# acrlabs/kube-scheduler-rs-reference

Measured on AMD Instinct MI355X. Metric: pod x node predicate evals/s, higher is better.
Workload: dtype int64

## Files before the change

kube_scheduler_rs_reference_amd/csrc/kernels_fused.hpp:

```cpp
#pragma once
#include <hip/hip_ext.h>
#include <hip/hip_runtime.h>
#include <stdint.h>

#include <type_traits>

#include "eval_request.hpp"
#include "kernarg.hpp"
#include "kernels_direct.hpp"
#include "tile_index.hpp"
#include "tile_launch.hpp"

#ifndef KSCHED_STORE_POLICY
#define KSCHED_STORE_POLICY 6
#endif
#ifndef KSCHED_STORE_ALT
#define KSCHED_STORE_ALT(it) ((it) == 7u)
#endif
#ifndef KSCHED_PROFILE
#define KSCHED_PROFILE 0
#endif
#if defined(KSCHED_FUSED_NUM_VGPR)
#define KSCHED_FUSED_WPE_ATTR __attribute__((amdgpu_num_vgpr(KSCHED_FUSED_NUM_VGPR)))
#elif defined(KSCHED_FUSED_WPE)
// ... 76 lines not shown
                if (eager == 1u) bnd = select_one_pod<5, 3>(sa, pod);
                else if (eager == 2u) bnd = select_one_pod<5, 5>(sa, pod);
                else if (eager == 3u) bnd = select_one_pod<5, 2>(sa, pod);
                else bnd = select_one_pod<5, 1>(sa, pod);
                sa.binding[pod] = bnd;
            }
            if (a.trace && threadIdx.x == 0u)
                atomicOr((unsigned long long *)&a.trace[(size_t)b * 8u + 7u], (unsigned long long)((wall_clock64() - t_in) << 8));
        }
        asm volatile("" : "+v"(tid) : : "memory");
    }
    const uint32_t lane = tid & 63u;
    const uint32_t wave = __builtin_amdgcn_readfirstlane(tid >> 6);
    const uint32_t stage_rank = (PICK == 1 && !(a.debug & 0x10000u)) ? wave - pick_waves : wave;
    const uint32_t stage_waves = kFusedWaves - pick_waves;
    const bool tracer = a.trace && tid == (PICK == 1 ? (kFusedWaves - 1u) * 64u : 0u);
    auto stamp = [&](uint32_t i) {
        if (tracer) a.trace[(size_t)b * 8u + i] = wall_clock64();
    };
    stamp(0);
    const uint32_t c_lo = chunk * a.unit_q + min(chunk, a.unit_rem);
    const uint32_t c_n = a.unit_q + (chunk < a.unit_rem ? 1u : 0u);
    uint32_t u = c_lo + (wave * c_n) / kFusedWaves;
    uint32_t u_hi = c_lo + ((wave + 1u) * c_n) / kFusedWaves;
    const uint32_t u_stride = a.u_stride;
    if (u_stride != 8u) {
        u = (a.wave_major ? wave * a.chunks + chunk : chunk * kFusedWaves + wave) * 8u;
        u_hi = a.units;
    }

    int64_t rc = 0, rm = 0;
    uint32_t s0 = 0, s1 = 0, s2 = 0, s3 = 0, s4 = 0, s5 = 0, s6 = 0, s7 = 0;
    uint64_t tol = 0;
    uint32_t d0 = 0, d1 = 0, d2 = 0, d3 = 0, d4 = 0;
    uint64_t ar = 0;
    auto issue_ops = [&](uint32_t pod) {
        const uint32_t pc = min(pod, a.p - 1u);
        if constexpr (PICK == 2) {
            static_assert(kPickAttempts == 5, "five draw registers");
            const size_t last = (size_t)a.p * kPickAttempts - 1u;
            const size_t f0 = (size_t)(pod - lane) * kPickAttempts + lane;
            asm volatile("global_load_dword %0, %1, off" : "=v"(d0) : "v"(sa.samples + min(f0, last)) : "memory");
            asm volatile("global_load_dword %0, %1, off" : "=v"(d1) : "v"(sa.samples + min(f0 + 64u, last)) : "memory");
            asm volatile("global_load_dword %0, %1, off" : "=v"(d2) : "v"(sa.samples + min(f0 + 128u, last)) : "memory");
            asm volatile("global_load_dword %0, %1, off" : "=v"(d3) : "v"(sa.samples + min(f0 + 192u, last)) : "memory");
            asm volatile("global_load_dword %0, %1, off" : "=v"(d4) : "v"(sa.samples + min(f0 + 256u, last)) : "memory");
        }
        if (FIT) {
            asm volatile("global_load_dwordx2 %0, %1, off" : "=v"(rc) : "v"(g_pcpu + pc) : "memory");
            asm volatile("global_load_dwordx2 %0, %1, off" : "=v"(rm) : "v"(g_pmem + pc) : "memory");
        }
        if (SEL) {
#define KSCHED_LOAD_SEL(K, DST)                                                                                                   \
    asm volatile("global_load_dword %0, %1, off"                                                                                  \
                 : "=v"(DST)                                                                                                      \
                 : "v"((uint32_t)K < a.nkeys ? g_psel + (size_t)K * a.p + pc : reinterpret_cast<const uint32_t *>(a.zero64)) \
                 : "memory")
            KSCHED_LOAD_SEL(0, s0);
            KSCHED_LOAD_SEL(1, s1);
            KSCHED_LOAD_SEL(2, s2);
            KSCHED_LOAD_SEL(3, s3);
            KSCHED_LOAD_SEL(4, s4);
            KSCHED_LOAD_SEL(5, s5);
            KSCHED_LOAD_SEL(6, s6);
            KSCHED_LOAD_SEL(7, s7);
#undef KSCHED_LOAD_SEL
        }
        if (TAINT) {
            const uint64_t *tp = a.has_tol ? g_ptol + pc : a.zero64;
            asm volatile("global_load_dwordx2 %0, %1, off" : "=v"(tol) : "v"(tp) : "memory");
        }
    };
#define KSCHED_WAIT_OPS(N)                                                                                                            \
    asm volatile("s_waitcnt vmcnt(%c11)"                                                                                              \
                 : "+v"(rc), "+v"(rm), "+v"(s0), "+v"(s1), "+v"(s2), "+v"(s3), "+v"(s4), "+v"(s5), "+v"(s6), "+v"(s7), "+v"(tol)  \
                 : "n"(N)                                                                                                             \
                 : "memory")
#define KSCHED_WAIT_OPS_PICK(N)                                                                                                       \
    asm volatile("s_waitcnt vmcnt(%c17)"                                                                                              \
                 : "+v"(rc), "+v"(rm), "+v"(s0), "+v"(s1), "+v"(s2), "+v"(s3), "+v"(s4), "+v"(s5), "+v"(s6), "+v"(s7), "+v"(tol), \
                   "+v"(d0), "+v"(d1), "+v"(d2), "+v"(d3), "+v"(d4), "+v"(ar)                                                     \
                 : "n"(N)                                                                                                             \
                 : "memory")
    const int64_t *s_cpu = reinterpret_cast<const int64_t *>(smem + a.off_aux);
    const int64_t *s_mem = s_cpu + kAuxTreeWords;
    const uint2 *s_cnt_cpu = reinterpret_cast<const uint2 *>(s_cpu + 2u * kAuxTreeWords);
    const uint2 *s_cnt_mem = s_cnt_cpu + kCntEntries;
    uint4 *s_fit = reinterpret_cast<uint4 *>(smem + a.off_fit) + wave * 64u;
    uint4 *s_lab = reinterpret_cast<uint4 *>(smem + a.off_lab) + wave * 64u;
    uint2 *s_trow = reinterpret_cast<uint2 *>(smem + a.off_trow) + wave * 64u;
    typedef __attribute__((address_space(3))) uint8_t lds_u8;
    lds_u8 *const lds = (lds_u8 *)smem;
    uint2 *s_lrec = reinterpret_cast<uint2 *>(smem + a.off_lrec) + wave * 64u;
    constexpr uint32_t kListCap = 8u;

    const uint32_t quad = (lane & 31u) >> 2;
    const uint32_t wp = ((0xCCu >> quad) & 1u) * 4u + (lane & 3u);
    const uint32_t sub = (lane >> 5) * 4u + ((0x31130220u >> (4u * quad)) & 15u);
    const uint32_t w0 = tile * kTileWords + 2u * wp;
    const bool has0 = w0 < a.pitch, has1 = w0 + 1u < a.pitch;
    const bool tile_full = (tile + 1u) * kTileWords <= a.pitch;
    const bool taint_inline = a.ngroups <= 4u;
    const uint8_t *Tb = smem + wp * 16u;
    const uint8_t *Tb_cpu = Tb + a.row_cpu * 128u;
    auto ldoff = [&](uint32_t off) -> u32x4 { return *reinterpret_cast<const u32x4 *>(Tb + off); };
    auto ldrow = [&](uint32_t row) -> u32x4 { return ldoff(row * 128u); };
    auto lo16 = [](uint32_t x) { return x & 0xFFFFu; };
    auto hi16 = [](uint32_t x) { return x >> 16; };
    const uint8_t *fit_lane = reinterpret_cast<const uint8_t *>(s_fit + sub) + wp;
    const uint2 *lab_lane = reinterpret_cast<const uint2 *>(s_lab + sub);
    const uint2 *trow_lane = s_trow + sub;
    auto opaque = [](uint32_t x) -> uint32_t {
        asm volatile("" : "+v"(x));
        return x;
    };
    auto lrec_of = [&](uint32_t it) -> uint2 { return (s_lrec + opaque(sub) + it * 8u)[0]; };
    auto list_mask = [&](uint32_t j, uint32_t rec, uint32_t bound, uint32_t wp) -> u32x4 {
        const uint32_t noff = a.off_list + j * kListBytes + kTileNodes * 4u;
        const uint32_t first = rec & 0xFFFFu, count = rec >> 16;
        u32x4 m = {0u, 0u, 0u, 0u};
        const uint32_t n_e = (bound != 0xFFFFFFFFu) ? bound : ((count == 0xFFFFu) ? 0u : count);
        for (uint32_t e = 0; e < n_e; ++e) {
            const uint32_t node = *(const __attribute__((address_space(3))) uint16_t *)(lds + noff + min(first + e, (uint32_t)kTileNodes - 1u) * 2u);
            const bool hit = e < count && (node >> 7) == wp;
            const uint32_t bit = hit ? (1u << (node & 31u)) : 0u, w = (node >> 5) & 3u;
            m.x |= (w == 0u) ? bit : 0u;
            m.y |= (w == 1u) ? bit : 0u;
            m.z |= (w == 2u) ? bit : 0u;
            m.w |= (w == 3u) ? bit : 0u;
        }
        const uint32_t all = (count == 0xFFFFu) ? 0xFFFFFFFFu : 0u;
        m.x |= all, m.y |= all, m.z |= all, m.w |= all;
        return m;
    };
    auto apply_lists = [&](u32x4 f, const uint2 lr, uint32_t bound) -> u32x4 {
        static_assert(kMaxListKeys == 2 && kListRecBytes == 8, "one 32-bit record slot per list key");
        const uint32_t r[2] = {lr.x, lr.y};
        const uint32_t wp_o = opaque(wp);
#pragma unroll
        for (uint32_t j = 0; j < 4; ++j)
            if (j < a.nlist) f &= list_mask(j, r[j], bound, wp_o);
        return f;
    };

    struct Rows {
        u32x4 c0, m0, l0, l1, l2, l3, t0, t1, t2, t3, x0, x1, x2, x3;
    };
    auto load_extra = [&](const uint2 r2, Rows &R) {
        R.x0 = ldoff(lo16(r2.x));
        R.x1 = ldoff(hi16(r2.x));
        R.x2 = ldoff(lo16(r2.y));
        R.x3 = ldoff(hi16(r2.y));
    };
    auto load_rows = [&](const uint32_t cc, const uint32_t cm, const uint2 lb, const uint2 tr, Rows &R) {
        if (FIT) {
            R.c0 = *reinterpret_cast<const u32x4 *>(Tb_cpu + cc * 128u);
            R.m0 = *reinterpret_cast<const u32x4 *>(Tb_cpu + cm * 128u + (uint32_t)kFitRows * 128u);
        } else {
            R.c0 = ldrow(a.row_valid);
        }
        if (SEL) {
            R.l0 = ldoff(lo16(lb.x));
            R.l1 = ldoff(hi16(lb.x));
            R.l2 = ldoff(lo16(lb.y));
            R.l3 = ldoff(hi16(lb.y));
        }
// ... 37 lines not shown
#elif KSCHED_STORE_POLICY == 2
        asm volatile("global_store_dwordx4 %0, %1, %2 sc1\n\ts_nop 1" ::"v"(voff), "v"(f), "s"(base) : "memory");
#elif KSCHED_STORE_POLICY == 3
        asm volatile("global_store_dwordx4 %0, %1, %2 sc0 sc1\n\ts_nop 1" ::"v"(voff), "v"(f), "s"(base) : "memory");
#elif KSCHED_STORE_POLICY == 4
        asm volatile("global_store_dwordx4 %0, %1, %2 sc1 nt\n\ts_nop 1" ::"v"(voff), "v"(f), "s"(base) : "memory");
#elif KSCHED_STORE_POLICY == 5
        asm volatile("global_store_dwordx4 %0, %1, %2 sc0 sc1 nt\n\ts_nop 1" ::"v"(voff), "v"(f), "s"(base) : "memory");
#elif KSCHED_STORE_POLICY == 1
        __builtin_nontemporal_store(f, reinterpret_cast<u32x4_a8 *>(reinterpret_cast<uint8_t *>(base) + voff));
#else
        *reinterpret_cast<u32x4_a8 *>(reinterpret_cast<uint8_t *>(base) + voff) = f;
#endif
    };
    auto uniform64 = [](uint64_t x) -> uint64_t {
        const uint32_t hi = (uint32_t)__builtin_amdgcn_readfirstlane((int)(uint32_t)(x >> 32)), lo = (uint32_t)__builtin_amdgcn_readfirstlane((int)(uint32_t)x);
        return ((uint64_t)hi << 32) | (uint64_t)lo;
    };
    uint64_t rb_feas = 0, rb_fit = 0;
    auto combine_store = [&](uint32_t it, const Rows &R, bool extra) {
        const uint64_t step = (uint64_t)it * step_bytes;
        u32x4 f = fit_of(R);
        if (WANT_FIT) store_rel(rb_fit + step, lane_off, f);
        if (SEL) f = ((f & R.l0) & R.l1) & (R.l2 & R.l3);
        if (SEL && extra) f = ((f & R.x0) & R.x1) & (R.x2 & R.x3);
        if (TAINT) f = ((f & R.t0) & R.t1) & (R.t2 & R.t3);
        store_rel(rb_feas + step, lane_off, f, KSCHED_STORE_ALT(it));
    };

    auto emit_checked = [&](uint32_t pod, uint32_t it, bool over) {
        const bool live = pod < a.p && has0;
        Rows R;
        if (LIST) {
            uint32_t sub_o = sub, wp_o = wp;
            asm volatile("" : "+v"(sub_o), "+v"(wp_o));
            const uint8_t *fit_o = reinterpret_cast<const uint8_t *>(s_fit + sub_o) + wp_o;
            const uint2 *lab_o = reinterpret_cast<const uint2 *>(s_lab + sub_o);
            load_rows(FIT ? (uint32_t)(fit_o + it * 128u)[0] : 0u, FIT ? (uint32_t)(fit_o + it * 128u)[8] : 0u, (lab_o + it * 16u)[0],
                      TAINT ? (s_trow + sub_o + it * 8u)[0] : make_uint2(0u, 0u), R);
            load_extra((lab_o + it * 16u)[1], R);
        } else {
            load_rows(rec_cc(it), rec_cm(it), rec_lb(it), rec_tr(it), R);
            if (SEL) load_extra(rec_lx(it), R);
        }
        u32x4 f = fit_of(R);
        const size_t o = (size_t)pod * a.pitch + w0;
        auto store = [&](uint64_t *dst) {
            if (has1) store16(dst, o, f);
            else dst[o] = ((uint64_t)f.y << 32) | f.x;
        };
        if (WANT_FIT && live) store(out_fit);
        if (SEL) {
            if (!over) {
                f = ((f & R.l0) & R.l1) & (R.l2 & R.l3);
                f = ((f & R.x0) & R.x1) & (R.x2 & R.x3);
            } else if (live) {
                for (uint32_t k = 0; k < a.nkeys; ++k) {
                    if (LIST && a.lab_meta[k] == kLabList) continue;
                    const uint32_t s = g_psel[(size_t)k * a.p + pod];
                    if (s != 0u) f &= ldrow((s <= a.lab_meta[32u + k]) ? (a.lab_meta[k] + s - 1u) : a.row_zero);
                }
            }
        }
        if (TAINT) {
            if (taint_inline) {
                f = ((f & R.t0) & R.t1) & (R.t2 & R.t3);
            } else if (live) {
                const uint64_t t = a.has_tol ? g_ptol[pod] : 0ull;
                for (uint32_t g = 0; g < a.ngroups; ++g) f &= ldrow(a.row_taint + 16u * g + (uint32_t)((t >> (4u * g)) & 15ull));
            }
        }
        if (LIST) {
            __builtin_amdgcn_sched_barrier(0);
            f = apply_lists(f, lrec_of(it), 0xFFFFFFFFu);
        }
        if (live && out_feas && !(a.debug & 1u)) store(out_feas);
    };

    bool extra_any = false, list_any = false;
    uint32_t list_bound = 0;
    uint32_t pick_bits = 0;
    typedef __attribute__((address_space(3))) uint32_t lds_u32;
    lds_u32 *const s_park = (lds_u32 *)(lds + a.off_park) + wave * (kPickAttempts * 64u);
    auto phase1 = [&](uint32_t pod0) -> uint64_t {
        uint2 cnt_c = make_uint2(0u, 0u), cnt_m = make_uint2(0u, 0u);
        if (FIT) {
            uint32_t lc = 0, lm = 0;
            if (!(a.debug & 2u)) {
                uint32_t kc = 1, km = 1;
#pragma unroll
                for (uint32_t level = 0; level < 10; ++level) {
                    const int64_t vc = s_cpu[kc], vm = s_mem[km];
                    kc = 2u * kc + ((vc < rc) ? 1u : 0u);
                    km = 2u * km + ((vm < rm) ? 1u : 0u);
                }
                lc = kc - (uint32_t)kTileNodes;
                lm = km - (uint32_t)kTileNodes;
                lc += (lc == (uint32_t)kTileNodes - 1u && s_cpu[0] < rc) ? 1u : 0u;
                lm += (lm == (uint32_t)kTileNodes - 1u && s_mem[0] < rm) ? 1u : 0u;
            }
            const uint2 cc = s_cnt_cpu[lc], cm = s_cnt_mem[lm];
            s_fit[lane] = make_uint4(cc.x, cc.y, cm.x, cm.y);
            cnt_c = cc;
            cnt_m = cm;
        }
        const uint32_t rv = a.row_valid * 128u;
        uint32_t cnt = 0;
        if (SEL) {
            const uint32_t rv2 = rv | (rv << 16);
            s_lab[lane] = make_uint4(rv2, rv2, rv2, rv2);
            uint16_t *const slots = reinterpret_cast<uint16_t *>(s_lab + lane);
            uint16_t *slot = slots;
            const uint32_t sv[8] = {s0, s1, s2, s3, s4, s5, s6, s7};
#pragma unroll
            for (uint32_t k = 0; k < 8; ++k) {
                const uint32_t s = sv[k];
                if (s != 0u && !(LIST && ((a.list_mask8 >> k) & 1u))) {
                    *slot++ = (uint16_t)(min(s, a.lab_mx1[k]) * 128u + a.lab_off[k]);
                }
            }
            cnt = (uint32_t)(slot - slots);
            if (a.nkeys > 8u) {
                const uint32_t pc = min(pod0 + lane, a.p - 1u);
                for (uint32_t k = 8; k < a.nkeys; ++k) {
                    if (LIST && a.lab_meta[k] == kLabList) continue;
                    cnt += (g_psel[(size_t)k * a.p + pc] != 0u) ? 9u : 0u;
                }
            }
        }
        uint32_t lmax = 0;
        if (LIST) {
            uint32_t lv[kMaxListKeys] = {0u, 0u};
#pragma unroll
            for (uint32_t j = 0; j < kMaxListKeys; ++j) {
                if (j >= a.nlist) continue;
                const uint32_t col = a.list_col[j];
                if (col < 8u) {
                    uint32_t v = s0;
                    v = (col == 1u) ? s1 : v;
                    v = (col == 2u) ? s2 : v;
                    v = (col == 3u) ? s3 : v;
                    v = (col == 4u) ? s4 : v;
                    v = (col == 5u) ? s5 : v;
                    v = (col == 6u) ? s6 : v;
                    v = (col == 7u) ? s7 : v;
                    lv[j] = v;
                } else {
                    lv[j] = g_psel[(size_t)col * a.p + min(pod0 + lane, a.p - 1u)];
                }
            }
            uint32_t rec[kMaxListKeys] = {0xFFFF0000u, 0xFFFF0000u};
            bool any = false;
#pragma unroll
            for (uint32_t j = 0; j < kMaxListKeys; ++j) {
                rec[j] = 0xFFFF0000u;
                const uint32_t s = lv[j];
                if (j < a.nlist && s != 0u) {
                    const uint32_t voff = a.off_list + j * kListBytes;
                    auto val_at = [&](uint32_t e) -> uint32_t { return *(const __attribute__((address_space(3))) uint32_t *)(lds + voff + e * 4u); };
                    auto lower = [&](uint32_t key) -> uint32_t {
                        uint32_t base = 0;
#pragma unroll
                        for (uint32_t half = (uint32_t)kTileNodes / 2u; half >= 1u; half >>= 1) base += (val_at(base + half - 1u) < key) ? half : 0u;
                        return base + ((val_at(base) < key) ? 1u : 0u);
                    };
                    const uint32_t lo = lower(s);
                    uint32_t cnt = 0;
                    bool run = true;
#pragma unroll
                    for (uint32_t e = 0; e <= kListCap; ++e) {
                        run = run && lo + e < (uint32_t)kTileNodes && val_at(min(lo + e, (uint32_t)kTileNodes - 1u)) == s;
                        cnt += run ? 1u : 0u;
                    }
                    if (cnt > kListCap) cnt = lower(s + 1u) - lo;
                    rec[j] = lo | (cnt << 16);
                    lmax = max(lmax, cnt);
                    any = true;
                }
            }
            s_lrec[lane] = make_uint2(rec[0], rec[1]);
            list_any = __ballot(any) != 0ull;
#pragma unroll
            for (uint32_t d = 32; d >= 1; d >>= 1) lmax = max(lmax, (uint32_t)__shfl_xor((int)lmax, d, 64));
            list_bound = (uint32_t)__builtin_amdgcn_readfirstlane((int)lmax);
        }
        if (TAINT) {
            uint32_t t[4];
#pragma unroll
            for (uint32_t g = 0; g < 4; ++g)
                t[g] = (g < a.ngroups) ? (a.row_taint + 16u * g + (uint32_t)((tol >> (4u * g)) & 15ull)) * 128u : rv;
            s_trow[lane] = make_uint2(t[0] | (t[1] << 16), t[2] | (t[3] << 16));
        }
        if constexpr (PICK == 2) {
            const uint4 slots = SEL ? s_lab[lane] : make_uint4(0u, 0u, 0u, 0u);
            s_park[lane] = d0;
            s_park[64u + lane] = d1;
            s_park[128u + lane] = d2;
            s_park[192u + lane] = d3;
            s_park[256u + lane] = d4;
            uint32_t dv[kPickAttempts];
#pragma unroll
            for (uint32_t i = 0; i < kPickAttempts; ++i) dv[i] = s_park[lane * kPickAttempts + i];
            uint32_t bits = 0;
#pragma unroll
            for (uint32_t i = 0; i < kPickAttempts; ++i) {
                const uint32_t l = dv[i] - tile * (uint32_t)kTileNodes;
                if (l < (uint32_t)kTileNodes && !(a.debug & 0x8000000u)) {
                    const uint32_t wofs = (l >> 5) << 2, sub = l >> 7;
                    auto word = [&](uint32_t off) -> uint32_t { return *(lds_u32 *)(lds + off + wofs); };
                    uint32_t v;
                    if (FIT) {
                        const uint32_t sh = (sub & 3u) * 8u;
                        const uint32_t bc = ((sub < 4u ? cnt_c.x : cnt_c.y) >> sh) & 0xFFu, bm = ((sub < 4u ? cnt_m.x : cnt_m.y) >> sh) & 0xFFu;
                        v = word((a.row_cpu + bc) * 128u) & word((a.row_cpu + (uint32_t)kFitRows + bm) * 128u);
                    } else {
                        v = word(rv);
                    }
                    if (SEL)
                        v &= word(slots.x & 0xFFFFu) & word(slots.x >> 16) & word(slots.y & 0xFFFFu) & word(slots.y >> 16) & word(slots.z & 0xFFFFu) &
                             word(slots.z >> 16) & word(slots.w & 0xFFFFu) & word(slots.w >> 16);
                    bits |= ((v >> (l & 31u)) & 1u) << i;
                }
            }
            pick_bits = bits;
        }
        extra_any = __ballot(cnt > 4u) != 0ull;
        const uint64_t over = __ballot(cnt > 8u || (LIST && lmax > kListCap));
        __builtin_amdgcn_fence(__ATOMIC_RELEASE, "wavefront");
        __builtin_amdgcn_wave_barrier();
        return over;
    };

    constexpr int kFastStores = 8 * (WANT_FIT ? 2 : 1);

    constexpr uint32_t kPrefetchRounds = 6;
    auto prefetch_rounds = [&]() {
        if (!(FIT || SEL || TAINT) || a.off_pf == 0xFFFFFFFFu || u + u_stride * (kPrefetchRounds + 2u) < u_hi || (a.debug & 0x20000000u)) return;
        const uint32_t dump = (uint32_t)__builtin_amdgcn_readfirstlane((int)a.off_pf);
        const uint32_t li = opaque(lane);
#pragma unroll 1
        for (uint32_t r = 1; r <= kPrefetchRounds; ++r) {
            const uint32_t pu = u + u_stride * r;
            if (pu >= u_hi) break;
            const uint32_t pod0 = pu * 8u;
            const uint32_t pe = a.p - 1u;
            const uint32_t e8 = min(pod0 + (li & 3u) * 16u, pe);
            uint64_t a64 = reinterpret_cast<uint64_t>(a.zero64);
            if (FIT && li < 4u) a64 = reinterpret_cast<uint64_t>(g_pcpu + e8);
            if (FIT && li >= 4u && li < 8u) a64 = reinterpret_cast<uint64_t>(g_pmem + e8);
            if (SEL && a.nkeys && li >= 8u && li < 24u) {
                const uint32_t k = min((li - 8u) >> 1, min(a.nkeys, 8u) - 1u);
                a64 = reinterpret_cast<uint64_t>(g_psel + (size_t)k * a.p + min(pod0 + (li & 1u) * 32u, pe));
            }
            if (PICK == 2 && li >= 24u && li < 34u) {
                a64 = reinterpret_cast<uint64_t>(sa.samples + min((size_t)pod0 * kPickAttempts + (li - 24u) * 32u, (size_t)a.p * kPickAttempts - 1u));
            }
            if (TAINT && a.has_tol && li >= 34u && li < 38u) {
                a64 = reinterpret_cast<uint64_t>(g_ptol + e8);
            }
            uint32_t m0_saved;
            asm volatile("s_mov_b32 %0, m0\n\ts_mov_b32 m0, %2\n\ts_nop 0\n\tglobal_load_lds_dword %1, off\n\ts_nop 0\n\ts_mov_b32 m0, %0\n\ts_nop 0" : "=&s"(m0_saved) : "v"(a64), "s"(dump) : "memory");
        }
    };
    bool more = u < u_hi, have_prev = false, first = true, stamped4 = false;
    uint32_t prev_u = 0, prev_nu = 0;
    uint64_t prev_over = 0;
    bool prev_extra = false, prev_list = false;
    uint32_t prev_bound = 0;
#if KSCHED_PROFILE
    uint64_t prof_p2 = 0, prof_wait = 0, prof_p1 = 0, prof_rounds = 0, prof_t = 0;
#define KSCHED_PROF(ACC)                                       \
    do {                                                       \
        const uint64_t now_ = __builtin_readcyclecounter();    \
        ACC += now_ - prof_t;                                  \
        prof_t = now_;                                         \
    } while (0)
#else
#define KSCHED_PROF(ACC) \
    do {                 \
    } while (0)
#endif
    auto pick_contribute = [&](uint32_t pod0, uint32_t nu) {
        const uint32_t n_live = min(nu * 8u, a.p - pod0);
        const uint32_t j = lane & 7u;
        uint32_t lo = 0, hi = 0;
        if (lane < n_live) {
            const uint64_t f = (uint64_t)pick_bits << (5u * j);
            lo = (uint32_t)f;
            hi = (uint32_t)(f >> 32);
        }
#pragma unroll
        for (uint32_t d = 1; d <= 4; d <<= 1) {
            lo |= (uint32_t)__shfl_xor((int)lo, (int)d, 64);
            hi |= (uint32_t)__shfl_xor((int)hi, (int)d, 64);
        }
        const uint64_t delta = (1ull << 40) | ((uint64_t)hi << 32) | (uint64_t)lo;
        uint64_t *const slot = a.pick_acc + ((pod0 >> 3) + (lane >> 3));
        const uint64_t lead = 0x0101010101010101ull & (n_live >= 64u ? ~0ull : ((1ull << n_live) - 1ull));
        uint64_t saved;
        asm volatile("s_and_saveexec_b64 %1, %4\n\tglobal_atomic_add_x2 %0, %2, %3, off sc0\n\ts_mov_b64 exec, %1"
                     : "=v"(ar), "=&s"(saved)
                     : "v"(slot), "v"(delta), "s"(lead)
                     : "memory", "scc");
    };
    auto pick_decide = [&](uint32_t pod0, uint32_t nu) {
        const uint32_t n_live = min(nu * 8u, a.p - pod0);
        const uint32_t j = lane & 7u, first = lane & ~7u;
        const uint32_t wlo = (uint32_t)__shfl((int)(uint32_t)ar, (int)first, 64), whi = (uint32_t)__shfl((int)(uint32_t)(ar >> 32), (int)first, 64);
        const uint64_t word = ((uint64_t)whi << 32) | (uint64_t)wlo;
        if (lane < n_live && (uint32_t)(word >> 40) == a.tiles - 1u) {
            const uint32_t all = ((uint32_t)(word >> (5u * j)) | pick_bits) & ((1u << kPickAttempts) - 1u);
            int32_t bnd = -1;
            if (all) bnd = (int32_t)s_park[lane * kPickAttempts + (uint32_t)__builtin_ctz(all)];
            sa.binding[pod0 + lane] = bnd;
            if (j == 0u) a.pick_acc[(pod0 >> 3) + (lane >> 3)] = 0ull;
        }
    };
    while (true) {
        if (PICK == 2 && have_prev && !(a.debug & 0x10000000u)) pick_contribute(prev_u * 8u, prev_nu);
        if (more) issue_ops(u * 8u + lane);
        if ((a.debug & 128u) && have_prev && !stamped4) stamp(1);
        if (first) {
            auto stage = [&](const void *gsrc, uint32_t lds_off, uint32_t bytes) {
                const uint8_t *g = static_cast<const uint8_t *>(gsrc);
                for (uint32_t off = stage_rank * 1024u; off < bytes; off += stage_waves * 1024u) {
                    if (off + lane * 16u < bytes)
                        __builtin_amdgcn_global_load_lds((const __attribute__((address_space(1))) void *)(g + off + lane * 16u),
                                                         (__attribute__((address_space(3))) void *)(lds + lds_off + off), 16, 0, 0);
                }
            };
            if (!pick_wave) {
                if (FIT) stage(g_aux + (size_t)tile * kAuxWords, a.off_aux, kAuxWords * 8u);
                if (LIST) stage(g_list + (size_t)tile * a.nlist * kListBytes, a.off_list, a.nlist * kListBytes);
                if (!(a.debug & 8u)) stage(g_tables + (size_t)tile * a.rows * kTileWords, 0u, a.rows * 128u);
            }
            if (!(a.debug & 128u)) stamp(1);
            if (PICK == 1) asm volatile("s_waitcnt vmcnt(0)" ::: "memory");
            __syncthreads();
            prefetch_rounds();
            if (!(a.debug & 128u)) stamp(2);
        }
        if (have_prev) {
#if KSCHED_PROFILE
            prof_t = __builtin_readcyclecounter();
#endif
            const uint32_t pod0 = prev_u * 8u;
            rb_feas = uniform64(reinterpret_cast<uint64_t>(out_feas + (size_t)pod0 * a.pitch));
            if (WANT_FIT) rb_fit = uniform64(reinterpret_cast<uint64_t>(out_fit + (size_t)pod0 * a.pitch));
            const bool fast = (prev_nu == 8u || !more) && prev_over == 0ull && pod0 + prev_nu * 8u <= a.p && tile_full &&
                              (!TAINT || taint_inline) && !(a.debug & 16u);
            if (LIST && fast && (prev_list || prev_nu != 8u)) {
                const uint32_t sub_o = opaque(sub), wp_o = opaque(wp);
                const uint8_t *fit_o = reinterpret_cast<const uint8_t *>(s_fit + sub_o) + wp_o;
                const uint2 *lab_o = reinterpret_cast<const uint2 *>(s_lab + sub_o);
                const uint2 *trow_o = s_trow + sub_o;
                Rows A;
                uint2 lr = (s_lrec + sub_o)[0];
                load_rows(FIT ? (uint32_t)fit_o[0] : 0u, FIT ? (uint32_t)fit_o[8] : 0u, lab_o[0], TAINT ? trow_o[0] : make_uint2(0u, 0u), A);
#pragma unroll 1
                for (uint32_t it = 0; it < prev_nu; ++it) {
                    const uint64_t step = (uint64_t)it * step_bytes;
                    u32x4 f = fit_of(A);
                    if (WANT_FIT) store_rel(rb_fit + step, lane_off, f);
                    f = ((f & A.l0) & A.l1) & (A.l2 & A.l3);
                    if (TAINT) f = ((f & A.t0) & A.t1) & (A.t2 & A.t3);
                    if (prev_extra) {
                        load_extra((lab_o + it * 16u)[1], A);
                        f = ((f & A.x0) & A.x1) & (A.x2 & A.x3);
                    }
                    const uint2 lr_now = lr;
                    const uint32_t nx = min(it + 1u, prev_nu - 1u);
                    __builtin_amdgcn_sched_barrier(0);
                    lr = (s_lrec + sub_o + nx * 8u)[0];
                    load_rows(FIT ? (uint32_t)(fit_o + nx * 128u)[0] : 0u, FIT ? (uint32_t)(fit_o + nx * 128u)[8] : 0u, (lab_o + nx * 16u)[0],
                              TAINT ? (trow_o + nx * 8u)[0] : make_uint2(0u, 0u), A);
                    f = apply_lists(f, lr_now, prev_bound);
                    store_rel(rb_feas + step, lane_off, f, KSCHED_STORE_ALT(it));
                }
            } else if (fast && prev_nu == 8u) {
                constexpr uint32_t STEP = TAINT ? 1u : 2u;
                uint32_t cn[STEP], mn[STEP];
                uint2 ln[STEP], tn[STEP];
#pragma unroll
                for (uint32_t j = 0; j < STEP; ++j) {
                    cn[j] = rec_cc(j);
                    mn[j] = rec_cm(j);
                    ln[j] = rec_lb(j);
                    tn[j] = rec_tr(j);
                }
                if (SEL && prev_extra) {
#pragma unroll
                    for (uint32_t it = 0; it < 8; ++it) {
                        Rows A;
                        const uint64_t step = (uint64_t)it * step_bytes;
                        load_rows(rec_cc(it), rec_cm(it), rec_lb(it), rec_tr(it), A);
                        u32x4 f = fit_of(A);
                        if (WANT_FIT) store_rel(rb_fit + step, lane_off, f);
                        f = ((f & A.l0) & A.l1) & (A.l2 & A.l3);
                        if (TAINT) f = ((f & A.t0) & A.t1) & (A.t2 & A.t3);
                        __builtin_amdgcn_sched_barrier(0);
                        load_extra(rec_lx(it), A);
                        f = ((f & A.x0) & A.x1) & (A.x2 & A.x3);
                        store_rel(rb_feas + step, lane_off, f, KSCHED_STORE_ALT(it));
                    }
                } else {
#pragma unroll
                    for (uint32_t it = 0; it < 8; it += STEP) {
                        Rows R[STEP];
#pragma unroll
                        for (uint32_t j = 0; j < STEP; ++j) load_rows(cn[j], mn[j], ln[j], tn[j], R[j]);
                        if (!TAINT && it + STEP < 8u) {
#pragma unroll
                            for (uint32_t j = 0; j < STEP; ++j) {
                                cn[j] = rec_cc(it + STEP + j);
                                mn[j] = rec_cm(it + STEP + j);
                                ln[j] = rec_lb(it + STEP + j);
                                tn[j] = rec_tr(it + STEP + j);
                            }
                        }
#pragma unroll
                        for (uint32_t j = 0; j < STEP; ++j) combine_store(it + j, R[j], false);
                        if (TAINT && it + STEP < 8u) {
#pragma unroll
                            for (uint32_t j = 0; j < STEP; ++j) {
                                cn[j] = rec_cc(it + STEP + j);
                                mn[j] = rec_cm(it + STEP + j);
                                ln[j] = rec_lb(it + STEP + j);
                                tn[j] = rec_tr(it + STEP + j);
                            }
                        }
                    }
                }
            } else if (!LIST && fast) {
#pragma unroll 1
                for (uint32_t it = 0; it < prev_nu; ++it) {
                    Rows A;
                    load_rows(rec_cc(it), rec_cm(it), rec_lb(it), rec_tr(it), A);
                    if (SEL) load_extra(rec_lx(it), A);
                    combine_store(it, A, true);
                }
            } else {
                if (!(a.debug & 16u)) {
#pragma unroll 1
                    for (uint32_t it = 0; it < prev_nu; ++it) {
                        const uint32_t pl = it * 8u + sub;
                        emit_checked(pod0 + pl, it, (prev_over >> pl) & 1ull);
                    }
                }
                asm volatile("s_waitcnt vmcnt(0)" ::: "memory");
            }
            if (!stamped4) stamp(4);
            stamped4 = true;
            __builtin_amdgcn_fence(__ATOMIC_ACQUIRE, "wavefront");
            __builtin_amdgcn_wave_barrier();
            KSCHED_PROF(prof_p2);
        }
        const bool had_more = more;
        if (more) {
#if KSCHED_PROFILE
            prof_t = __builtin_readcyclecounter();
            ++prof_rounds;
#endif
            if constexpr (PICK == 2) {
                KSCHED_WAIT_OPS_PICK(kFastStores);
                if (have_prev) pick_decide(prev_u * 8u, prev_nu);
            } else {
                KSCHED_WAIT_OPS(kFastStores);
            }
            KSCHED_PROF(prof_wait);
            prev_over = phase1(u * 8u);
            KSCHED_PROF(prof_p1);
            prev_extra = extra_any;
            prev_list = list_any;
            prev_bound = list_bound;
            if (!have_prev) stamp(3);
            prev_u = u;
            prev_nu = min(8u, u_hi - u);
            have_prev = true;
            u += u_stride;
            more = u < u_hi;
        }
        if (PICK == 2 && !had_more && have_prev) {
            asm volatile("s_waitcnt vmcnt(0)" : "+v"(ar) : : "memory");
            pick_decide(prev_u * 8u, prev_nu);
        }
        first = false;
        if (!had_more) break;
    }
#undef KSCHED_WAIT_OPS
#undef KSCHED_WAIT_OPS_PICK
    if (a.trace && lane == 0) {
        atomicMax((unsigned long long *)&a.trace[(size_t)b * 8u + 5u], (unsigned long long)wall_clock64());
        __builtin_amdgcn_s_waitcnt(0);
        atomicMax((unsigned long long *)&a.trace[(size_t)b * 8u + 6u], (unsigned long long)wall_clock64());
    }
#if KSCHED_PROFILE
    if (tracer) {
        a.trace[(size_t)b * 8u + 1u] = prof_p2;
        a.trace[(size_t)b * 8u + 2u] = prof_wait;
        a.trace[(size_t)b * 8u + 3u] = prof_p1;
        a.trace[(size_t)b * 8u + 4u] = prof_rounds;
    }
#endif
#undef KSCHED_PROF
    if (tracer) {
        uint32_t xcc;
        asm volatile("s_getreg_b32 %0, hwreg(HW_REG_XCC_ID)" : "=s"(xcc));
        atomicOr((unsigned long long *)&a.trace[(size_t)b * 8u + 7u], (unsigned long long)(xcc & 0xFFu));
    }
}

struct FusedLaunch {
    dim3 grid;
    uint32_t lds;
    hipStream_t stream;
    const IndexedSnapshot *snap;
    const int64_t *pcpu, *pmem;
    const uint32_t *psel;
    const uint64_t *ptol;
    uint64_t *out_feas, *out_fit;
    hipEvent_t ev_start, ev_stop;
    const SelectArgs *pick;
    int pick_form;
};

template <bool FIT, bool SEL, bool TAINT, bool WANT_FIT, bool LIST, int PICK = 0>
inline hipError_t launch_fused_k(const FusedLaunch &q, const FusedArgs &a) {
    auto kern = k_eval_fused<FIT, SEL, TAINT, WANT_FIT, LIST, PICK>;
    hipError_t e = hipFuncSetAttribute((const void *)kern, hipFuncAttributeMaxDynamicSharedMemorySize, (int)q.lds);
    if (e != hipSuccess) return e;
    const IndexedSnapshot &s = *q.snap;
    const SelectArgs sa = q.pick ? *q.pick : SelectArgs{};
    if (q.ev_start || q.ev_stop)
        hipExtLaunchKernelGGL(kern, q.grid, dim3(kFusedThreads), q.lds, q.stream, q.ev_start, q.ev_stop, 0, s.d_tables, s.d_aux, q.pcpu,
                              q.pmem, q.psel, q.ptol, q.out_feas, q.out_fit, (const uint8_t *)s.d_list, a, sa);
    else
        hipLaunchKernelGGL(kern, q.grid, dim3(kFusedThreads), q.lds, q.stream, s.d_tables, s.d_aux, q.pcpu, q.pmem, q.psel, q.ptol,
                           q.out_feas, q.out_fit, (const uint8_t *)s.d_list, a, sa);
    return hipGetLastError();
}

template <bool FIT, bool SEL, bool TAINT>
inline hipError_t launch_fused_t(bool want_fit, bool list, const FusedLaunch &q, const FusedArgs &a) {
    if constexpr (SEL) {
        if (list) return want_fit ? launch_fused_k<FIT, SEL, TAINT, true, true>(q, a) : launch_fused_k<FIT, SEL, TAINT, false, true>(q, a);
    }
    if (q.pick && !want_fit) {
        if constexpr (!TAINT) {
            if (q.pick_form == 2) return launch_fused_k<FIT, SEL, TAINT, false, false, 2>(q, a);
        }
        return launch_fused_k<FIT, SEL, TAINT, false, false, 1>(q, a);
    }
    return want_fit ? launch_fused_k<FIT, SEL, TAINT, true, false>(q, a) : launch_fused_k<FIT, SEL, TAINT, false, false>(q, a);
}

inline bool fused_pick_applicable(const IndexedSnapshot &s, const TileTerms &t, uint32_t p) {
    return s.built && !t.want_fit && !t.list && p < (1u << 31);
}
inline bool fused_tile_pick_applicable(const IndexedLayout &l, const TileTerms &t, uint32_t attempts) {
    if (attempts != kPickAttempts || t.taint) return false;
    if (t.sel && l.nkeys > 8u) return false;
    return tile_lds_layout(l, lds_want(t, true)).bytes <= kLdsBudget;
}

inline bool fused_applicable(const IndexedSnapshot &s, const TileTerms &t) {
    return s.built && tile_lds_layout(s.lay, lds_want(t, false)).bytes <= kLdsBudget;
}

struct FusedOptions {
    uint32_t debug = 0;
    hipEvent_t ev_start = nullptr, ev_stop = nullptr;
    uint64_t *trace = nullptr;
    uint32_t trace_blocks = 0;
// ... 44 lines not shown
```

kube_scheduler_rs_reference_amd/csrc/tile_launch.hpp:

```cpp
#pragma once

#include <algorithm>
#include <type_traits>

#include "eval_request.hpp"
#include "tile_index.hpp"

#ifndef KSCHED_FUSED_THREADS
#define KSCHED_FUSED_THREADS 1024
#endif

namespace ksched {

constexpr uint32_t kFusedThreads = KSCHED_FUSED_THREADS;
constexpr uint32_t kFusedWaves = kFusedThreads / 64;

struct TileTerms {
    bool fit, sel, taint;
    bool list;
    bool want_fit;
};

inline TileTerms tile_terms(const EvalRequest &r, const IndexedLayout &l) {
    const bool sel = r.sel(l.nkeys);
    return TileTerms{r.fit(), sel, r.taint(l.ngroups != 0), sel && l.nlist > 0, r.want_fit()};
}

constexpr uint32_t kLdsFit = 1u, kLdsSel = 2u, kLdsTaint = 4u;
constexpr uint32_t kLdsPark = 8u;
constexpr uint32_t kLdsPrefetch = 16u;
constexpr uint32_t kLdsEveryRegion = kLdsFit | kLdsSel | kLdsTaint;

constexpr uint32_t kPickAttempts = 5;
constexpr uint32_t kPickParkBytes = kFusedWaves * kPickAttempts * 64u * 4u;
constexpr uint32_t kPrefetchDumpBytes = 256u;

struct TileLds {
    uint32_t off_aux, off_fit, off_lab, off_trow, off_list, off_lrec, off_park;
    uint32_t off_pf;
    uint32_t bytes;
};

constexpr uint32_t lds_want(const TileTerms &t, bool park) {
    return (t.fit ? kLdsFit : 0u) | (t.sel ? kLdsSel : 0u) | (t.taint ? kLdsTaint : 0u) | (park ? kLdsPark : 0u) | kLdsPrefetch;
}

constexpr TileLds tile_lds_layout(const IndexedLayout &l, uint32_t want) {
    constexpr uint32_t pods = kFusedWaves * 64u;
    const bool lists = (want & kLdsSel) && l.nlist;
    uint32_t off = l.rows * 128u;
    auto take = [&off](bool on, uint32_t bytes) {
        const uint32_t at = off;
        if (on) off += bytes;
        return at;
    };
    TileLds d{};
    d.off_aux = take(want & kLdsFit, kAuxWords * 8u);
    d.off_fit = take(want & kLdsFit, pods * 16u);
    d.off_lab = take(want & kLdsSel, pods * 16u);
    d.off_trow = take(want & kLdsTaint, pods * 8u);
    d.off_list = take(lists, l.nlist * kListBytes);
    d.off_lrec = take(lists, pods * kListRecBytes);
    d.off_park = take(want & kLdsPark, kPickParkBytes);
    d.off_pf = (want & kLdsPrefetch) && off + kPrefetchDumpBytes <= kLdsBudget ? take(true, kPrefetchDumpBytes) : 0xFFFFFFFFu;
    d.bytes = off;
    return d;
}

constexpr bool lds_is_what_indexed_plan_checks(uint32_t nlist) {
    IndexedLayout l{};
    l.nlist = nlist;
    return tile_lds_layout(l, kLdsEveryRegion).bytes == lds_non_row_bytes(nlist);
}
static_assert(lds_is_what_indexed_plan_checks(0) && lds_is_what_indexed_plan_checks(1) && lds_is_what_indexed_plan_checks(kMaxListKeys),
              "tile_lds_layout and indexed_plan's LDS budget have drifted apart");

inline uint32_t resident_blocks_per_cu(uint32_t lds) { return std::max(1u, std::min(kLdsBudget / lds, 2048u / kFusedThreads)); }

struct FusedGeometryIn {
    uint32_t p = 0, tiles = 1;
    uint32_t lds = 0;
    bool pick = false;
    uint32_t grid_cus = 0;
    int round_order = 0;
    uint32_t debug = 0;
};

struct FusedGeometry {
    uint32_t units, chunks, unit_q, unit_rem;
    uint32_t u_stride, wave_major;
    uint32_t tiles_rcp, run, grid;
    uint32_t pick_ppb, pick_waves;
};

inline FusedGeometry fused_geometry(const FusedGeometryIn &in) {
    FusedGeometry g{};
    g.units = (in.p + 7u) / 8u;
    const uint32_t blocks_per_cu = resident_blocks_per_cu(in.lds);
    const uint32_t rounds = (g.units + 7u) / 8u;
    uint32_t per_block = kFusedWaves;
    if (in.pick) per_block = 4u;
    if (((in.debug >> 18) & 3u) == 1u) per_block = kFusedWaves;
    if (((in.debug >> 18) & 3u) == 2u) per_block = 4u;
    if (((in.debug >> 18) & 3u) == 3u) per_block = 1u;
    const uint32_t want = (rounds + per_block - 1u) / per_block;
    const uint32_t cus = in.grid_cus ? std::min(256u, in.grid_cus) : 256u;
    g.chunks = std::max(1u, std::min((cus * blocks_per_cu) / in.tiles, want));
    if (in.round_order != 1 && !(in.debug & 0x80000000u)) {
        const uint32_t streams = g.chunks * kFusedWaves;
        const uint32_t per_wave = (rounds + streams - 1u) / streams;
        if (per_wave == 2u) g.chunks = std::max(1u, std::min(g.chunks, (rounds + 2u * kFusedWaves - 1u) / (2u * kFusedWaves)));
    }
    g.unit_q = g.units / g.chunks;
    g.unit_rem = g.units % g.chunks;
    g.u_stride = in.round_order == 1 ? 8u : g.chunks * kFusedWaves * 8u;
    g.wave_major = in.round_order == 2 ? 0u : 1u;
    g.tiles_rcp = (uint32_t)std::min<uint64_t>((1ull << 32) / in.tiles, 0xFFFFFFFFull);
    const uint32_t total = g.chunks * in.tiles;
    g.run = (total + 7u) / 8u;
    g.grid = (in.debug & 32u) ? total : g.run * 8u;
    if (in.pick) {
        g.pick_ppb = (in.p + total - 1u) / total;
        g.pick_waves = std::max(1u, std::min(8u, (g.pick_ppb + 63u) / 64u));
    }
    return g;
}

struct SummaryGeometry {
    uint32_t rounds, chunks, grid;
};

inline SummaryGeometry summary_geometry(uint32_t p, uint32_t tiles, uint32_t lds) {
    SummaryGeometry g{};
    g.rounds = (p + 63u) / 64u;
    g.chunks = std::max(1u, std::min((256u * resident_blocks_per_cu(lds)) / tiles, (g.rounds + kFusedWaves - 1u) / kFusedWaves));
    g.grid = g.chunks * tiles;
    return g;
}

template <class Args>
inline void fill_tile_args(Args &a, const IndexedSnapshot &s, const TileLds &d, const TileTerms &t, const EvalRequest &r) {
    const IndexedLayout &l = s.lay;
    a.p = r.p;
    a.tiles = l.tiles;
    a.rows = l.rows;
    a.nkeys = l.nkeys;
    a.ngroups = l.ngroups;
    a.row_zero = l.row_zero;
    a.row_valid = l.row_valid;
    a.row_cpu = l.row_cpu;
    a.row_taint = l.row_taint;
    for (int k = 0; k < 8; ++k) {
        const bool is_list = l.lab_base[k] == kLabList;
        a.lab_off[k] = is_list ? 0u : (l.lab_base[k] - 1u) * 128u;
        a.lab_mx1[k] = is_list ? 0u : l.lab_max[k] + 1u;
    }
    a.lab_meta = s.d_lab_meta;
    a.zero64 = reinterpret_cast<const uint64_t *>(s.d_lab_meta + 64);
// ... 23 lines not shown
```

Before: 25750 billion.

## Precompute first-round label slots and pick parking before the staging barrier

On the first loop trip, each wave waits only for its own operand loads using a counted vmcnt switch keyed to how many staging pieces it issued. It then writes the label-slot records and parks the pick candidates in LDS before the __syncthreads, so this work overlaps the barrier wait instead of running after it. phase1 gains a compile-time PRE path that reuses the precomputed count and local node indices. The change adds inline-asm LDS writes, a counted-wait switch that depends on staging-piece bookkeeping staying consistent, and some extra code size.

Result: slower. 25100 billion (-2.5%).

```diff
diff --git a/kube_scheduler_rs_reference_amd/csrc/kernels_fused.hpp b/kube_scheduler_rs_reference_amd/csrc/kernels_fused.hpp
--- a/kube_scheduler_rs_reference_amd/csrc/kernels_fused.hpp
+++ b/kube_scheduler_rs_reference_amd/csrc/kernels_fused.hpp
@@ -182,6 +182,24 @@
                    "+v"(d0), "+v"(d1), "+v"(d2), "+v"(d3), "+v"(d4), "+v"(ar)                                                     \
                  : "n"(N)                                                                                                             \
                  : "memory")
+#define KSCHED_WAIT_STAGED_CASE(N)                                                              \
+    case N:                                                                                     \
+        asm volatile("s_waitcnt vmcnt(" #N ") ; first round: operands landed" ::: "memory");    \
+        break
+#define KSCHED_NAME_STAGED()                                                                                                                   \
+    do {                                                                                                                                       \
+        if constexpr (PICK == 2)                                                                                                               \
+            asm volatile("; first round: operands named"                                                                                       \
+                         : "+v"(rc), "+v"(rm), "+v"(s0), "+v"(s1), "+v"(s2), "+v"(s3), "+v"(s4), "+v"(s5), "+v"(s6), "+v"(s7), "+v"(tol),      \
+                           "+v"(d0), "+v"(d1), "+v"(d2), "+v"(d3), "+v"(d4)                                                                    \
+                         :                                                                                                                     \
+                         : "memory");                                                                                                          \
+        else                                                                                                                                   \
+            asm volatile("; first round: operands named"                                                                                       \
+                         : "+v"(rc), "+v"(rm), "+v"(s0), "+v"(s1), "+v"(s2), "+v"(s3), "+v"(s4), "+v"(s5), "+v"(s6), "+v"(s7), "+v"(tol)       \
+                         :                                                                                                                     \
+                         : "memory");                                                                                                          \
+    } while (0)
     const int64_t *s_cpu = reinterpret_cast<const int64_t *>(smem + a.off_aux);
     const int64_t *s_mem = s_cpu + kAuxTreeWords;
     const uint2 *s_cnt_cpu = reinterpret_cast<const uint2 *>(s_cpu + 2u * kAuxTreeWords);
@@ -385,7 +403,12 @@
     uint32_t pick_bits = 0;
     typedef __attribute__((address_space(3))) uint32_t lds_u32;
     lds_u32 *const s_park = (lds_u32 *)(lds + a.off_park) + wave * (kPickAttempts * 64u);
-    auto phase1 = [&](uint32_t pod0) -> uint64_t {
+    struct PreRound {
+        uint32_t cnt;
+        uint32_t l[kPickAttempts];
+    };
+    auto phase1 = [&](uint32_t pod0, auto pre_c, const PreRound pre) -> uint64_t {
+        constexpr bool PRE = decltype(pre_c)::value;
         uint2 cnt_c = make_uint2(0u, 0u), cnt_m = make_uint2(0u, 0u);
         if (FIT) {
             uint32_t lc = 0, lm = 0;
@@ -410,19 +433,23 @@
         const uint32_t rv = a.row_valid * 128u;
         uint32_t cnt = 0;
         if (SEL) {
-            const uint32_t rv2 = rv | (rv << 16);
-            s_lab[lane] = make_uint4(rv2, rv2, rv2, rv2);
-            uint16_t *const slots = reinterpret_cast<uint16_t *>(s_lab + lane);
-            uint16_t *slot = slots;
-            const uint32_t sv[8] = {s0, s1, s2, s3, s4, s5, s6, s7};
-#pragma unroll
-            for (uint32_t k = 0; k < 8; ++k) {
-                const uint32_t s = sv[k];
-                if (s != 0u && !(LIST && ((a.list_mask8 >> k) & 1u))) {
-                    *slot++ = (uint16_t)(min(s, a.lab_mx1[k]) * 128u + a.lab_off[k]);
-                }
-            }
-            cnt = (uint32_t)(slot - slots);
+            if constexpr (PRE) {
+                cnt = pre.cnt;
+            } else {
+                const uint32_t rv2 = rv | (rv << 16);
+                s_lab[lane] = make_uint4(rv2, rv2, rv2, rv2);
+                uint16_t *const slots = reinterpret_cast<uint16_t *>(s_lab + lane);
+                uint16_t *slot = slots;
+                const uint32_t sv[8] = {s0, s1, s2, s3, s4, s5, s6, s7};
+#pragma unroll
+                for (uint32_t k = 0; k < 8; ++k) {
+                    const uint32_t s = sv[k];
+                    if (s != 0u && !(LIST && ((a.list_mask8 >> k) & 1u))) {
+                        *slot++ = (uint16_t)(min(s, a.lab_mx1[k]) * 128u + a.lab_off[k]);
+                    }
+                }
+                cnt = (uint32_t)(slot - slots);
+            }
             if (a.nkeys > 8u) {
                 const uint32_t pc = min(pod0 + lane, a.p - 1u);
                 for (uint32_t k = 8; k < a.nkeys; ++k) {
@@ -496,18 +523,23 @@
         }
         if constexpr (PICK == 2) {
             const uint4 slots = SEL ? s_lab[lane] : make_uint4(0u, 0u, 0u, 0u);
-            s_park[lane] = d0;
-            s_park[64u + lane] = d1;
-            s_park[128u + lane] = d2;
-            s_park[192u + lane] = d3;
-            s_park[256u + lane] = d4;
-            uint32_t dv[kPickAttempts];
-#pragma unroll
-            for (uint32_t i = 0; i < kPickAttempts; ++i) dv[i] = s_park[lane * kPickAttempts + i];
+            uint32_t dl[kPickAttempts];
+            if constexpr (PRE) {
+#pragma unroll
+                for (uint32_t i = 0; i < kPickAttempts; ++i) dl[i] = pre.l[i];
+            } else {
+                s_park[lane] = d0;
+                s_park[64u + lane] = d1;
+                s_park[128u + lane] = d2;
+                s_park[192u + lane] = d3;
+                s_park[256u + lane] = d4;
+#pragma unroll
+                for (uint32_t i = 0; i < kPickAttempts; ++i) dl[i] = s_park[lane * kPickAttempts + i] - tile * (uint32_t)kTileNodes;
+            }
             uint32_t bits = 0;
 #pragma unroll
             for (uint32_t i = 0; i < kPickAttempts; ++i) {
-                const uint32_t l = dv[i] - tile * (uint32_t)kTileNodes;
+                const uint32_t l = dl[i];
                 if (l < (uint32_t)kTileNodes && !(a.debug & 0x8000000u)) {
                     const uint32_t wofs = (l >> 5) << 2, sub = l >> 7;
                     auto word = [&](uint32_t off) -> uint32_t { return *(lds_u32 *)(lds + off + wofs); };
@@ -535,6 +567,8 @@
     };
 
     constexpr int kFastStores = 8 * (WANT_FIT ? 2 : 1);
+    constexpr bool kPrep = !TAINT && !LIST && !WANT_FIT && PICK != 1 && (SEL || PICK == 2);
+    constexpr uint32_t kDebugNoPrep = 0x2000000u;
 
     constexpr uint32_t kPrefetchRounds = 6;
     auto prefetch_rounds = [&]() {
@@ -616,13 +650,16 @@
             int32_t bnd = -1;
             if (all) bnd = (int32_t)s_park[lane * kPickAttempts + (uint32_t)__builtin_ctz(all)];
             sa.binding[pod0 + lane] = bnd;
-            if (j == 0u) a.pick_acc[(pod0 >> 3) + (lane >> 3)] = 0ull;
+            const uint32_t z = opaque(0u);
+            if (j == 0u) a.pick_acc[(pod0 >> 3) + (lane >> 3)] = ((uint64_t)z << 32) | (uint64_t)z;
         }
     };
     while (true) {
         if (PICK == 2 && have_prev && !(a.debug & 0x10000000u)) pick_contribute(prev_u * 8u, prev_nu);
         if (more) issue_ops(u * 8u + lane);
         if ((a.debug & 128u) && have_prev && !stamped4) stamp(1);
+        bool prepped = false;
+        PreRound pre{};
         if (first) {
             auto stage = [&](const void *gsrc, uint32_t lds_off, uint32_t bytes) {
                 const uint8_t *g = static_cast<const uint8_t *>(gsrc);
@@ -638,6 +675,71 @@
                 if (!(a.debug & 8u)) stage(g_tables + (size_t)tile * a.rows * kTileWords, 0u, a.rows * 128u);
             }
             if (!(a.debug & 128u)) stamp(1);
+            if constexpr (kPrep) {
+                if (more && !(a.debug & kDebugNoPrep)) {
+                    const uint32_t n_st = (FIT ? stage_pieces(kAuxWords * 8u, wave, kFusedWaves) : 0u) +
+                                          ((a.debug & 8u) ? 0u : stage_pieces(a.rows * 128u, wave, kFusedWaves)) +
+                                          ((a.trace && wave == 0u && !(a.debug & 128u)) ? 1u : 0u);
+                    if (n_st <= kMaxStagePieces + 1u) {
+                        static_assert(kMaxStagePieces + 1u == 15u, "one switch arm per count");
+                        switch (n_st) {
+                            KSCHED_WAIT_STAGED_CASE(0);
+                            KSCHED_WAIT_STAGED_CASE(1);
+                            KSCHED_WAIT_STAGED_CASE(2);
+                            KSCHED_WAIT_STAGED_CASE(3);
+                            KSCHED_WAIT_STAGED_CASE(4);
+                            KSCHED_WAIT_STAGED_CASE(5);
+                            KSCHED_WAIT_STAGED_CASE(6);
+                            KSCHED_WAIT_STAGED_CASE(7);
+                            KSCHED_WAIT_STAGED_CASE(8);
+                            KSCHED_WAIT_STAGED_CASE(9);
+                            KSCHED_WAIT_STAGED_CASE(10);
+                            KSCHED_WAIT_STAGED_CASE(11);
+                            KSCHED_WAIT_STAGED_CASE(12);
+                            KSCHED_WAIT_STAGED_CASE(13);
+                            KSCHED_WAIT_STAGED_CASE(14);
+                            KSCHED_WAIT_STAGED_CASE(15);
+                        }
+                        KSCHED_NAME_STAGED();
+                        const uint32_t lds0 = (uint32_t)(uintptr_t)lds;
+                        if (SEL) {
+                            const uint32_t rv_ = a.row_valid * 128u, rv2 = rv_ | (rv_ << 16);
+                            const uint32_t rec = lds0 + a.off_lab + (wave * 64u + lane) * 16u;
+                            const u32x4 fill = {rv2, rv2, rv2, rv2};
+                            asm volatile("ds_write_b128 %0, %1\n\ts_nop 1" ::"v"(rec), "v"(fill) : "memory");
+                            const uint32_t sv[8] = {s0, s1, s2, s3, s4, s5, s6, s7};
+                            uint32_t n = 0;
+#pragma unroll
+                            for (uint32_t k = 0; k < 8; ++k) {
+                                const uint32_t s = sv[k];
+                                const uint32_t row = s != 0u ? min(s, a.lab_mx1[k]) * 128u + a.lab_off[k] : rv_;
+                                asm volatile("ds_write_b16 %0, %1" ::"v"(rec + 2u * n), "v"(row) : "memory");
+                                n += s != 0u ? 1u : 0u;
+                            }
+                            pre.cnt = n;
+                        }
+                        if constexpr (PICK == 2) {
+                            const uint32_t park = lds0 + a.off_park + wave * (kPickAttempts * 64u * 4u);
+                            uint32_t t0, t1, t2, t3, t4;
+                            asm volatile(
+                                "ds_write_b32 %5, %7\n\tds_write_b32 %5, %8 offset:256\n\tds_write_b32 %5, %9 offset:512\n\t"
+                                "ds_write_b32 %5, %10 offset:768\n\tds_write_b32 %5, %11 offset:1024\n\t"
+                                "ds_read_b32 %0, %6\n\tds_read_b32 %1, %6 offset:4\n\tds_read_b32 %2, %6 offset:8\n\t"
+                                "ds_read_b32 %3, %6 offset:12\n\tds_read_b32 %4, %6 offset:16\n\ts_waitcnt lgkmcnt(0)"
+                                : "=&v"(t0), "=&v"(t1), "=&v"(t2), "=&v"(t3), "=&v"(t4)
+                                : "v"(park + lane * 4u), "v"(park + lane * (kPickAttempts * 4u)), "v"(d0), "v"(d1), "v"(d2), "v"(d3), "v"(d4)
+                                : "memory");
+                            const uint32_t first_node = tile * (uint32_t)kTileNodes;
+                            pre.l[0] = t0 - first_node;
+                            pre.l[1] = t1 - first_node;
+                            pre.l[2] = t2 - first_node;
+                            pre.l[3] = t3 - first_node;
+                            pre.l[4] = t4 - first_node;
+                        }
+                        prepped = true;
+                    }
+                }
+            }
             if (PICK == 1) asm volatile("s_waitcnt vmcnt(0)" ::: "memory");
             __syncthreads();
             prefetch_rounds();
@@ -771,7 +873,12 @@
                 KSCHED_WAIT_OPS(kFastStores);
             }
             KSCHED_PROF(prof_wait);
-            prev_over = phase1(u * 8u);
+            if constexpr (kPrep) {
+                if (prepped) prev_over = phase1(u * 8u, std::true_type{}, pre);
+                else prev_over = phase1(u * 8u, std::false_type{}, PreRound{});
+            } else {
+                prev_over = phase1(u * 8u, std::false_type{}, PreRound{});
+            }
             KSCHED_PROF(prof_p1);
             prev_extra = extra_any;
             prev_list = list_any;
@@ -792,6 +899,8 @@
     }
 #undef KSCHED_WAIT_OPS
 #undef KSCHED_WAIT_OPS_PICK
+#undef KSCHED_NAME_STAGED
+#undef KSCHED_WAIT_STAGED_CASE
     if (a.trace && lane == 0) {
         atomicMax((unsigned long long *)&a.trace[(size_t)b * 8u + 5u], (unsigned long long)wall_clock64());
         __builtin_amdgcn_s_waitcnt(0);
diff --git a/kube_scheduler_rs_reference_amd/csrc/tile_launch.hpp b/kube_scheduler_rs_reference_amd/csrc/tile_launch.hpp
--- a/kube_scheduler_rs_reference_amd/csrc/tile_launch.hpp
+++ b/kube_scheduler_rs_reference_amd/csrc/tile_launch.hpp
@@ -74,6 +74,14 @@
 }
 static_assert(lds_is_what_indexed_plan_checks(0) && lds_is_what_indexed_plan_checks(1) && lds_is_what_indexed_plan_checks(kMaxListKeys),
               "tile_lds_layout and indexed_plan's LDS budget have drifted apart");
+
+constexpr uint32_t stage_pieces(uint32_t bytes, uint32_t rank, uint32_t waves) {
+    const uint32_t n = (bytes + 1023u) / 1024u;
+    return n > rank ? (n - rank + waves - 1u) / waves : 0u;
+}
+constexpr uint32_t kMaxStagePieces = 14;
+static_assert(kFusedWaves < 16u || stage_pieces(kAuxWords * 8u, 0u, kFusedWaves) + stage_pieces(kLdsBudget, 0u, kFusedWaves) <= kMaxStagePieces,
+              "a wave can issue more staging pieces than the first trip's counted wait has forms for");
 
 inline uint32_t resident_blocks_per_cu(uint32_t lds) { return std::max(1u, std::min(kLdsBudget / lds, 2048u / kFusedThreads)); }
 
```
